# RS2002/PianoBart

Measured on AMD Instinct MI355X. Metric: Octuple tokens/sec/GPU (seq=1024, 12L/768d) pretrain step; %MFMA peak, higher is better.
Workload: dtype bf16

## Files before the change

pianobart_amd/csrc/pb_fa_tiles.h:

```cpp
#pragma once
#include "pb_common.h"
#include "pb_api_internal.h"

namespace {


constexpr int HD = 64, FT = 256;
constexpr float LOG2E = 1.4426950408889634f;
typedef __attribute__((ext_vector_type(4))) short s16x4;
typedef __attribute__((ext_vector_type(8))) short s16x8;

struct Fa64Args {
    const bf16_t *q, *k, *v, *o, *dout;
    bf16_t *out, *dq, *dk, *dv;
    float* lse; const float* delta; const float* key_mask; const int* kmax;
    int B, H, Sq, Sk;
    long q_sb, q_ss, k_sb, k_ss, v_sb, v_ss, o_sb, o_ss, dq_sb, dq_ss, dk_sb, dk_ss, dv_sb, dv_ss;
    float scale; int causal;
    float* cs_q; float* cs_kv;
    const bf16_t* zeros;
    const int *vl_q_off, *vl_k_off, *vl_q_len, *vl_k_len;
    const int* bh_order;
};

inline Fa64Args fa64_args(const pb_attn_desc& d, bool bwd) {
    Fa64Args a = {};
    a.q = (const bf16_t*)d.q; a.k = (const bf16_t*)d.k; a.v = (const bf16_t*)d.v; a.dout = (const bf16_t*)d.dout;
    if (bwd) a.o = (const bf16_t*)d.o; else a.out = (bf16_t*)d.o;
    a.dq = (bf16_t*)d.dq; a.dk = (bf16_t*)d.dk; a.dv = (bf16_t*)d.dv; a.lse = d.lse; a.delta = d.delta;
    a.key_mask = d.key_mask; a.kmax = d.q_off ? d.k_vis : d.kmax;
    a.B = d.B; a.H = d.H; a.Sq = d.Sq; a.Sk = d.Sk;
    a.q_sb = d.q_sb; a.q_ss = d.q_ss; a.k_sb = d.k_sb; a.k_ss = d.k_ss; a.v_sb = d.v_sb; a.v_ss = d.v_ss; a.o_sb = d.o_sb; a.o_ss = d.o_ss;
    a.dq_sb = d.dq_sb; a.dq_ss = d.dq_ss; a.dk_sb = d.dk_sb; a.dk_ss = d.dk_ss; a.dv_sb = d.dv_sb; a.dv_ss = d.dv_ss;
    a.scale = d.scale; a.causal = d.flags & PB_ATTN_CAUSAL;
    a.zeros = (const bf16_t*)pb_zero_page();
    a.vl_q_off = d.q_off; a.vl_k_off = d.k_off; a.vl_q_len = d.q_len; a.vl_k_len = d.k_len; a.bh_order = d.bh_order;
    return a;
}

__device__ __forceinline__ void varlen_localize(Fa64Args& p, int b) {
    if (!p.vl_q_off) return;
    const long qo = p.vl_q_off[b], ko = p.vl_k_off[b];
    p.Sq = p.vl_q_len[b]; p.Sk = p.vl_k_len[b];
    p.q += qo * p.q_ss - b * p.q_sb; p.k += ko * p.k_ss - b * p.k_sb; p.v += ko * p.v_ss - b * p.v_sb;
    if (p.o) p.o += qo * p.o_ss - b * p.o_sb;
    if (p.out) p.out += qo * p.o_ss - b * p.o_sb;
    if (p.dout) p.dout += qo * p.o_ss - b * p.o_sb;
    if (p.dq) p.dq += qo * p.dq_ss - b * p.dq_sb;
    if (p.dk) p.dk += ko * p.dk_ss - b * p.dk_sb;
    if (p.dv) p.dv += ko * p.dv_ss - b * p.dv_sb;
}

#define MFMA16(a, b, c) __builtin_amdgcn_mfma_f32_16x16x32_bf16((a), (b), (c), 0, 0, 0)

__device__ __forceinline__ int fsw(int row) { return (((row >> 1) & 3) << 1) | ((row >> 3) & 1); }

__device__ __forceinline__ void glds16(const bf16_t* g, char* lds_wave_base) {
    __builtin_amdgcn_global_load_lds((const __attribute__((address_space(1))) void*)g,
                                     (__attribute__((address_space(3))) void*)lds_wave_base, 16, 0, 0);
}
struct StageOff { unsigned off[2]; unsigned chunk[2]; };
__device__ __forceinline__ StageOff stage_off(long ld, int wave, int lane) {
    StageOff o;
#pragma unroll
    for (int n = 0; n < 2; ++n) {
        const int row = (wave * 2 + n) * 8 + (lane >> 3);
        o.chunk[n] = (unsigned)((lane & 7) ^ fsw(row));
        o.off[n] = (unsigned)(row * ld + (o.chunk[n] << 3));
    }
    return o;
}
__device__ __forceinline__ void stage64(const bf16_t* __restrict__ base, long ld, int r0, int nrows, char* lds, int wave, int lane, const StageOff& so,
                                        int cmax = 8, const bf16_t* zeros = nullptr) {
    if (r0 + 64 <= nrows) {
        const bf16_t* tb = base + (long)r0 * ld;
#pragma unroll
        for (int n = 0; n < 2; ++n) glds16((cmax == 8 || (int)so.chunk[n] < cmax) ? tb + so.off[n] : zeros, lds + (wave * 2 + n) * 1024);
    } else {
#pragma unroll
        for (int n = 0; n < 2; ++n) {
            const int inst = wave * 2 + n;
            const int row = inst * 8 + (lane >> 3);
            const int chunk = (lane & 7) ^ fsw(row);
            const int gr = min(r0 + row, nrows - 1);
            glds16((cmax == 8 || chunk < cmax) ? base + (long)gr * ld + chunk * 8 : zeros, lds + inst * 1024);
        }
    }
}
__device__ __forceinline__ bf16x8 frag_row(const char* lds, int row, int ks, int g) {
    return *reinterpret_cast<const bf16x8*>(lds + row * 128 + (((ks * 4 + g) ^ fsw(row)) << 4));
}
__device__ __forceinline__ bf16x8 frag_tr(const char* lds, int c0, int s, int lane) {
    const int lr = lane & 15, g = lane >> 4, qq = lr >> 2, pp = lr & 3;
    const int chunk = (c0 >> 3) + (pp >> 1);
    const int r0 = 32 * s + 4 * g + qq, r1 = r0 + 16;
    const int o0 = r0 * 128 + ((chunk ^ fsw(r0)) << 4) + ((pp & 1) << 3);
    const int o1 = r1 * 128 + ((chunk ^ fsw(r1)) << 4) + ((pp & 1) << 3);
    const s16x4 lo = __builtin_amdgcn_ds_read_tr16_b64_v4i16((__attribute__((address_space(3))) s16x4*)(lds + o0));
    const s16x4 hi = __builtin_amdgcn_ds_read_tr16_b64_v4i16((__attribute__((address_space(3))) s16x4*)(lds + o1));
    const s16x8 v = {lo[0], lo[1], lo[2], lo[3], hi[0], hi[1], hi[2], hi[3]};
    return __builtin_bit_cast(bf16x8, v);
}
__device__ __forceinline__ bf16x8 pack_pair(const f32x4& lo, const f32x4& hi) {
    bf16x8 r = {(bf16_t)lo[0], (bf16_t)lo[1], (bf16_t)lo[2], (bf16_t)lo[3], (bf16_t)hi[0], (bf16_t)hi[1], (bf16_t)hi[2], (bf16_t)hi[3]};
    return r;
}
__device__ __forceinline__ bf16x8 frag_global(const bf16_t* __restrict__ g, long ld, int row, int nvalid, int col) {
    bf16x8 z = {};
    if (row < nvalid) z = *reinterpret_cast<const bf16x8*>(g + (long)row * ld + col);
    return z;
}
__device__ __forceinline__ float grp_max(float v) {
    auto a = __builtin_amdgcn_permlane16_swap(__float_as_uint(v), __float_as_uint(v), false, false);
    v = fmaxf(__uint_as_float(a[0]), __uint_as_float(a[1]));
    auto b = __builtin_amdgcn_permlane32_swap(__float_as_uint(v), __float_as_uint(v), false, false);
    return fmaxf(__uint_as_float(b[0]), __uint_as_float(b[1]));
}
__device__ __forceinline__ float grp_sum(float v) {
    auto a = __builtin_amdgcn_permlane16_swap(__float_as_uint(v), __float_as_uint(v), false, false);
    v = __uint_as_float(a[0]) + __uint_as_float(a[1]);
    auto b = __builtin_amdgcn_permlane32_swap(__float_as_uint(v), __float_as_uint(v), false, false);
    return __uint_as_float(b[0]) + __uint_as_float(b[1]);
}
template <bool V> struct BoolTag { static constexpr bool value = V; };

constexpr int STG = 2 * 8192 + 512;
// ... 54 lines not shown
```

pianobart_amd/csrc/pb_flash1.hip:

```cpp
#include "pb_common.h"
#include "pb_fa_tiles.h"
#include <cstdlib>
#include <algorithm>

namespace {

constexpr int KB1 = 256;
constexpr int RING1 = 3, STB1 = 2 * 8192;
constexpr int OFF_K = RING1 * STB1;
constexpr int OFF_DS = OFF_K + 4 * 8192;
constexpr int OFF_TAB = OFF_DS + 2 * 2 * 8192;

struct Fa1Args {
    Fa64Args a;
    bf16_t* slab;
    long slab_stride, slab_sb;
    const float* delta_rows; long delta_ld;
    unsigned* stamps;
};

#define PB_U10(p) p "0", p "1", p "2", p "3", p "4", p "5", p "6", p "7", p "8", p "9"
#define PB_ALL_AGPRS PB_U10("a"), PB_U10("a1"), PB_U10("a2"), PB_U10("a3"), PB_U10("a4"), PB_U10("a5"), PB_U10("a6"), PB_U10("a7"), PB_U10("a8"), PB_U10("a9"), \
    PB_U10("a10"), PB_U10("a11"), PB_U10("a12"), PB_U10("a13"), PB_U10("a14"), PB_U10("a15"), PB_U10("a16"), PB_U10("a17"), PB_U10("a18"), PB_U10("a19"), \
    PB_U10("a20"), PB_U10("a21"), PB_U10("a22"), PB_U10("a23"), PB_U10("a24"), "a250", "a251", "a252", "a253", "a254", "a255"
constexpr int A_DK = 0, A_DV = 64, A_KF = 128, A_VF = 160, A_KT = 192;
typedef __attribute__((ext_vector_type(4))) unsigned u32x4;

template <int R> __device__ __forceinline__ void agpr_zero() { asm volatile("v_accvgpr_write_b32 a%c0, 0" :: "i"(R)); }
template <int R> __device__ __forceinline__ void agpr_put(const bf16x8& v) {
    const u32x4 u = __builtin_bit_cast(u32x4, v);
    asm volatile("v_accvgpr_write_b32 a%c4, %0\n\tv_accvgpr_write_b32 a%c5, %1\n\tv_accvgpr_write_b32 a%c6, %2\n\tv_accvgpr_write_b32 a%c7, %3"
                 :: "v"(u[0]), "v"(u[1]), "v"(u[2]), "v"(u[3]), "i"(R), "i"(R + 1), "i"(R + 2), "i"(R + 3));
}
template <int R> __device__ __forceinline__ f32x4 agpr_get() {
    f32x4 r;
    asm volatile("v_accvgpr_read_b32 %0, a%c4\n\tv_accvgpr_read_b32 %1, a%c5\n\tv_accvgpr_read_b32 %2, a%c6\n\tv_accvgpr_read_b32 %3, a%c7"
                 : "=v"(r[0]), "=v"(r[1]), "=v"(r[2]), "=v"(r[3]) : "i"(R), "i"(R + 1), "i"(R + 2), "i"(R + 3));
    return r;
}
template <int RB> __device__ __forceinline__ void mfma_vab_c(f32x4& d, const bf16x8& a, const f32x4& c) {
    asm volatile("v_mfma_f32_16x16x32_bf16 %0, %1, a[%c3:%c4], %2" : "=&v"(d) : "v"(a), "v"(c), "i"(RB), "i"(RB + 3) : PB_ALL_AGPRS);
}
template <int RB> __device__ __forceinline__ void mfma_vab(f32x4& d, const bf16x8& a) {
    asm volatile("v_mfma_f32_16x16x32_bf16 %0, %1, a[%c2:%c3], %0" : "+v"(d) : "v"(a), "i"(RB), "i"(RB + 3) : PB_ALL_AGPRS);
}
template <int RA> __device__ __forceinline__ void mfma_aav(f32x4& d, const bf16x8& b) {
    asm volatile("v_mfma_f32_16x16x32_bf16 %0, a[%c2:%c3], %1, %0" : "+v"(d) : "v"(b), "i"(RA), "i"(RA + 3) : PB_ALL_AGPRS);
}
template <int RA> __device__ __forceinline__ void mfma_aav_z(f32x4& d, const bf16x8& b) {
    asm volatile("v_mfma_f32_16x16x32_bf16 %0, a[%c2:%c3], %1, 0" : "=&v"(d) : "v"(b), "i"(RA), "i"(RA + 3) : PB_ALL_AGPRS);
}
template <int RD> __device__ __forceinline__ void mfma_acc(const bf16x8& b, const bf16x8& a) {
    asm volatile("v_mfma_f32_16x16x32_bf16 a[%c2:%c3], %0, %1, a[%c2:%c3]" :: "v"(a), "v"(b), "i"(RD), "i"(RD + 3) : PB_ALL_AGPRS);
}
#define MF "v_mfma_f32_16x16x32_bf16 "
template <int DT, int K0> __device__ __forceinline__ void mfma_dvdk4(const bf16x8& p0, const bf16x8& d0, const bf16x8& p1, const bf16x8& d1, const bf16x8& ot, const bf16x8& qt) {
    asm volatile(MF "a[%c6:%c7], %4, %0, a[%c6:%c7]\n\t" MF "a[%c8:%c9], %5, %1, a[%c8:%c9]\n\t" MF "a[%c10:%c11], %4, %2, a[%c10:%c11]\n\t" MF "a[%c12:%c13], %5, %3, a[%c12:%c13]"
                 :: "v"(p0), "v"(d0), "v"(p1), "v"(d1), "v"(ot), "v"(qt),
                    "i"(A_DV + 4 * (K0 * 4 + DT)), "i"(A_DV + 4 * (K0 * 4 + DT) + 3), "i"(A_DK + 4 * (K0 * 4 + DT)), "i"(A_DK + 4 * (K0 * 4 + DT) + 3),
                    "i"(A_DV + 4 * ((K0 + 1) * 4 + DT)), "i"(A_DV + 4 * ((K0 + 1) * 4 + DT) + 3), "i"(A_DK + 4 * ((K0 + 1) * 4 + DT)), "i"(A_DK + 4 * ((K0 + 1) * 4 + DT) + 3)
                 : PB_ALL_AGPRS);
}
template <int KT> __device__ __forceinline__ void mfma_sdp0(f32x4& sv, f32x4& dp, const bf16x8& qa, const bf16x8& oa, const f32x4& nl, const f32x4& nd) {
    asm volatile(MF "%0, %2, a[%c6:%c7], %4\n\t" MF "%1, %3, a[%c8:%c9], %5"
                 : "=&v"(sv), "=&v"(dp) : "v"(qa), "v"(oa), "v"(nl), "v"(nd),
                   "i"(A_KF + 4 * (KT * 2)), "i"(A_KF + 4 * (KT * 2) + 3), "i"(A_VF + 4 * (KT * 2)), "i"(A_VF + 4 * (KT * 2) + 3) : PB_ALL_AGPRS);
}
template <int KT> __device__ __forceinline__ void mfma_sdp1(f32x4& sv, f32x4& dp, const bf16x8& qa, const bf16x8& oa) {
    asm volatile(MF "%0, %2, a[%c4:%c5], %0\n\t" MF "%1, %3, a[%c6:%c7], %1"
                 : "+v"(sv), "+v"(dp) : "v"(qa), "v"(oa),
                   "i"(A_KF + 4 * (KT * 2 + 1)), "i"(A_KF + 4 * (KT * 2 + 1) + 3), "i"(A_VF + 4 * (KT * 2 + 1)), "i"(A_VF + 4 * (KT * 2 + 1) + 3) : PB_ALL_AGPRS);
}
template <int S0, bool ZERO> __device__ __forceinline__ void mfma_dq4(f32x4& a0, f32x4& b0, f32x4& a1, f32x4& b1, const bf16x8& bs0, const bf16x8& bs1) {
    if constexpr (ZERO)
        asm volatile(MF "%0, a[%c6:%c7], %4, 0\n\t" MF "%1, a[%c8:%c9], %4, 0\n\t" MF "%2, a[%c10:%c11], %5, 0\n\t" MF "%3, a[%c12:%c13], %5, 0"
                     : "=&v"(a0), "=&v"(b0), "=&v"(a1), "=&v"(b1) : "v"(bs0), "v"(bs1),
                       "i"(A_KT + 4 * S0), "i"(A_KT + 4 * S0 + 3), "i"(A_KT + 4 * (8 + S0)), "i"(A_KT + 4 * (8 + S0) + 3),
                       "i"(A_KT + 4 * (S0 + 1)), "i"(A_KT + 4 * (S0 + 1) + 3), "i"(A_KT + 4 * (9 + S0)), "i"(A_KT + 4 * (9 + S0) + 3) : PB_ALL_AGPRS);
    else
        asm volatile(MF "%0, a[%c6:%c7], %4, %0\n\t" MF "%1, a[%c8:%c9], %4, %1\n\t" MF "%2, a[%c10:%c11], %5, %2\n\t" MF "%3, a[%c12:%c13], %5, %3"
                     : "+v"(a0), "+v"(b0), "+v"(a1), "+v"(b1) : "v"(bs0), "v"(bs1),
                       "i"(A_KT + 4 * S0), "i"(A_KT + 4 * S0 + 3), "i"(A_KT + 4 * (8 + S0)), "i"(A_KT + 4 * (8 + S0) + 3),
                       "i"(A_KT + 4 * (S0 + 1)), "i"(A_KT + 4 * (S0 + 1) + 3), "i"(A_KT + 4 * (9 + S0)), "i"(A_KT + 4 * (9 + S0) + 3) : PB_ALL_AGPRS);
}
#undef MF
template <int OFF, class T> __device__ __forceinline__ void ds_rd128(T& d, unsigned addr) {
    static_assert(sizeof(T) == 16, "16-byte fragment");
    asm volatile("ds_read_b128 %0, %1 offset:%2" : "=v"(d) : "v"(addr), "i"(OFF));
}
__device__ __forceinline__ bf16x4 to_bf4(const f32x4& v) {
    bf16x4 r = {(bf16_t)v[0], (bf16_t)v[1], (bf16_t)v[2], (bf16_t)v[3]};
    return r;
}
__device__ __forceinline__ bf16x8 join4(const bf16x4& lo, const bf16x4& hi) { return __builtin_shufflevector(lo, hi, 0, 1, 2, 3, 4, 5, 6, 7); }
#define PB_PIN() __builtin_amdgcn_sched_barrier(0)

__global__ __launch_bounds__(FT) void fa1_bwd_kernel(const Fa1Args pin) {
    constexpr int HDT = 64;
    extern __shared__ __attribute__((aligned(16))) char smem[];
    const int t = threadIdx.x, lane = t & 63, lr = lane & 15, g = lane >> 4;
    const int wave = __builtin_amdgcn_readfirstlane(t >> 6);
#ifdef PB_FA1_STAMPS
    const unsigned long long st_in = __builtin_amdgcn_s_memrealtime();
#endif
    const int nkb0 = (pin.a.Sk + KB1 - 1) / KB1;
    int rb, h, b;
    block_map(nkb0, pin.a.H, pin.a.B, rb, h, b, pin.a.bh_order);
    const int k0 = rb * KB1;
    Fa64Args p = pin.a;
    const long qrow0 = pin.a.vl_q_off ? (long)pin.a.vl_q_off[b] : (long)b * pin.a.Sq;
    varlen_localize(p, b);
    const int lse_ld = pin.a.Sq, d_model = p.H * HDT;
    const int kvis_end = p.kmax ? min(p.Sk, p.kmax[b]) : p.Sk;
    const int nt = (p.Sq + 63) / 64;
    const int it0 = p.causal ? k0 / 64 : 0;
    const bf16_t* K = p.k + b * p.k_sb + h * HDT;
    const bf16_t* V = p.v + b * p.v_sb + h * HDT;
    if (k0 >= kvis_end || it0 >= nt) {
        for (int i = t; i < KB1 * 8; i += FT) {
            const int key = k0 + (i >> 3), ch = i & 7;
            if (key < p.Sk) {
                const bf16x8 z = {};
                *reinterpret_cast<bf16x8*>(p.dk + b * p.dk_sb + (long)key * p.dk_ss + h * HDT + ch * 8) = z;
                *reinterpret_cast<bf16x8*>(p.dv + b * p.dv_sb + (long)key * p.dv_ss + h * HDT + ch * 8) = z;
            }
        }
        if (p.cs_kv && t < 2 * HDT) {
            float* row = p.cs_kv + (long)(b * nkb0 + rb) * 2 * d_model + h * HDT;
            row[t < HDT ? t : d_model + t - HDT] = 0.f;
        }
        return;
    }
    asm volatile("" ::: PB_ALL_AGPRS);
#ifdef PB_FA1_STAMPS
    const unsigned st_t0 = (unsigned)__builtin_amdgcn_s_memtime();
    unsigned st_p[6] = {}, st_q[4] = {};
#define PSTAMP(i) st_p[i] = (unsigned)__builtin_amdgcn_s_memtime();
#define QSTAMP(i) st_q[i] = (unsigned)__builtin_amdgcn_s_memtime();
#else
#define PSTAMP(i)
#define QSTAMP(i)
#endif
    const bf16_t* Q = p.q + b * p.q_sb + h * HDT;
    const bf16_t* DO = p.dout + b * p.o_sb + h * HDT;
    bf16_t* slab = pin.slab + (long)rb * pin.slab_stride + (pin.a.vl_q_off ? qrow0 * d_model : (long)b * pin.slab_sb) + h * HDT;
    const float c = p.scale * LOG2E;
    bf16x8 kfr[4][2], vfr[4][2];
#pragma unroll
    for (int kt = 0; kt < 4; ++kt) {
        const int key = k0 + wave * 64 + kt * 16 + lr;
#pragma unroll
        for (int ks = 0; ks < 2; ++ks) {
            kfr[kt][ks] = frag_global(K, p.k_ss, key, p.Sk, ks * 32 + g * 8);
            vfr[kt][ks] = frag_global(V, p.v_ss, key, p.Sk, ks * 32 + g * 8);
        }
    }
    QSTAMP(0);
    float* ldsNL = reinterpret_cast<float*>(smem + OFF_TAB);
    float* ldsND = ldsNL + nt * 64;
    float* ldsVis = reinterpret_cast<float*>(smem + OFF_DS);
    const long li0 = ((long)b * p.H + h) * lse_ld;
    const float* dsrc = pin.delta_rows ? pin.delta_rows + (long)h * pin.delta_ld + qrow0 : p.delta + li0;
    float tl[4], td[4];
#pragma unroll
    for (int i = 0; i < 4; ++i) {
        const int q = it0 * 64 + t + i * FT;
        tl[i] = q < p.Sq ? p.lse[li0 + q] : INFINITY;
        td[i] = q < p.Sq ? dsrc[q] : 0.f;
    }
    QSTAMP(1);
    const int key_t = k0 + t;
    const float vis_t = (key_t < kvis_end && (!p.key_mask || p.key_mask[(long)b * p.Sk + key_t] != 0.f)) ? 1.f : 0.f;
    const StageOff so_k = stage_off(p.k_ss, wave, lane), so_q = stage_off(p.q_ss, wave, lane), so_o = stage_off(p.o_ss, wave, lane);
    const __amdgpu_buffer_rsrc_t rsK = __builtin_amdgcn_make_buffer_rsrc(const_cast<bf16_t*>(K), 0, (int)(((long)(p.Sk - 1) * p.k_ss + HDT) * 2), 0x00020000);
    const __amdgpu_buffer_rsrc_t rsQ = __builtin_amdgcn_make_buffer_rsrc(const_cast<bf16_t*>(Q), 0, (int)(((long)(p.Sq - 1) * p.q_ss + HDT) * 2), 0x00020000);
    const __amdgpu_buffer_rsrc_t rsO = __builtin_amdgcn_make_buffer_rsrc(const_cast<bf16_t*>(DO), 0, (int)(((long)(p.Sq - 1) * p.o_ss + HDT) * 2), 0x00020000);
    const __amdgpu_buffer_rsrc_t rsS = __builtin_amdgcn_make_buffer_rsrc(slab, 0, (int)(((long)(p.Sq - 1) * d_model + HDT) * 2), 0x00020000);
    const unsigned stg = lds_u32(smem) + OFF_K + (unsigned)(wave * 1024);
    const unsigned stg_wa = stg + (unsigned)(lr * 64 + ((((g >> 1) ^ ((lr >> 1) & 3)) << 4) | ((g & 1) << 3)));
    const unsigned stg_wb = stg + (unsigned)(lr * 64 + (((2 + (g >> 1)) ^ ((lr >> 1) & 3)) << 4 | ((g & 1) << 3)));
    const int srow = lane >> 2, schunk = lane & 3;
    const unsigned stg_rd = stg + (unsigned)(srow * 64 + ((schunk ^ ((srow >> 1) & 3)) << 4));
    const unsigned slab_vo = (unsigned)((((wave & 1) * 16 + srow) * d_model + (wave >> 1) * 32 + schunk * 8) * 2);
    u32x4 slab_v = {0u, 0u, 0u, 0u};
    int slab_qs = 0;
    bool slab_pending = false;
    typedef __attribute__((ext_vector_type(2))) unsigned u32x2_t;
    auto slab_put = [&](const f32x4& a, const f32x4& b_, int qs) {
        *reinterpret_cast<__attribute__((address_space(3))) u32x2_t*>(stg_wa) = __builtin_bit_cast(u32x2_t, to_bf4(a));
        *reinterpret_cast<__attribute__((address_space(3))) u32x2_t*>(stg_wb) = __builtin_bit_cast(u32x2_t, to_bf4(b_));
        ds_rd128<0>(slab_v, stg_rd);
        slab_qs = qs; slab_pending = true;
    };
    auto slab_flush = [&]() {
        if (slab_pending) { __builtin_amdgcn_raw_buffer_store_b128(slab_v, rsS, slab_vo, slab_qs, 0); slab_pending = false; }
    };
    const unsigned voQ0 = so_q.off[0] * 2, voQ1 = so_q.off[1] * 2, voO0 = so_o.off[0] * 2, voO1 = so_o.off[1] * 2;
    typedef __attribute__((address_space(3))) void* lds_t;
#pragma unroll
    for (int m = 0; m < 4; ++m) {
        const int sk = (k0 + 64 * m) * (int)p.k_ss * 2;
        __builtin_amdgcn_raw_ptr_buffer_load_lds(rsK, (lds_t)(smem + OFF_K + m * 8192 + wave * 2048), 16, so_k.off[0] * 2, sk, 0, 0);
        __builtin_amdgcn_raw_ptr_buffer_load_lds(rsK, (lds_t)(smem + OFF_K + m * 8192 + wave * 2048 + 1024), 16, so_k.off[1] * 2, sk, 0, 0);
    }
    auto stage = [&](int it, int slot) {
        char* st = smem + slot * STB1 + wave * 2048;
        const int sq = it * 64 * (int)p.q_ss * 2, so = it * 64 * (int)p.o_ss * 2;
        __builtin_amdgcn_raw_ptr_buffer_load_lds(rsQ, (lds_t)st, 16, voQ0, sq, 0, 0);
        __builtin_amdgcn_raw_ptr_buffer_load_lds(rsQ, (lds_t)(st + 1024), 16, voQ1, sq, 0, 0);
        __builtin_amdgcn_raw_ptr_buffer_load_lds(rsO, (lds_t)(st + 8192), 16, voO0, so, 0, 0);
        __builtin_amdgcn_raw_ptr_buffer_load_lds(rsO, (lds_t)(st + 8192 + 1024), 16, voO1, so, 0, 0);
    };
    QSTAMP(2);
    const int npre = min(3, nt - it0);
    stage(it0, 0);
    if (npre > 1) stage(it0 + 1, 1);
    if (npre > 2) stage(it0 + 2, 2);
    PSTAMP(0);
#pragma unroll
    for (int i = 0; i < 4; ++i) {
        const int q = it0 * 64 + t + i * FT;
        if (q < nt * 64) { ldsNL[q] = tl[i] == INFINITY ? -INFINITY : -tl[i] * LOG2E; ldsND[q] = -td[i]; }
    }
    for (int q = it0 * 64 + t + 4 * FT; q < nt * 64; q += FT) {
        const float ls = q < p.Sq ? p.lse[li0 + q] : INFINITY;
        ldsNL[q] = ls == INFINITY ? -INFINITY : -ls * LOG2E;
        ldsND[q] = q < p.Sq ? -dsrc[q] : 0.f;
    }
    ldsVis[t] = vis_t;
    bool hot = false;
#pragma unroll
    for (int i = 0; i < 4; ++i) hot |= (tl[i] != INFINITY && -tl[i] * LOG2E > 100.f);
    for (int q = it0 * 64 + t + 4 * FT; q < p.Sq; q += FT) hot |= (-p.lse[li0 + q] * LOG2E > 100.f);
    unsigned* ldsHot = reinterpret_cast<unsigned*>(smem + OFF_DS + 1024);
    const unsigned hotw = __builtin_amdgcn_ballot_w64(hot) != 0ull ? 1u : 0u;
    if (lane == 0) ldsHot[wave] = hotw;
    PSTAMP(1);
    bool allvis = true;
    static_for<0, 4>([&](auto ktt) {
        constexpr int kt = decltype(ktt)::value;
        const int key = k0 + wave * 64 + kt * 16 + lr;
        const bool vis = key < kvis_end && (!p.key_mask || p.key_mask[(long)b * p.Sk + key] != 0.f);
        allvis &= vis;
        static_for<0, 2>([&](auto kss) {
            constexpr int ks = decltype(kss)::value;
            bf16x8 kf = scale_frag(kfr[kt][ks], c);
            const bf16x8 z = {};
            if (!vis) kf = z;
            agpr_put<A_KF + 4 * (kt * 2 + ks)>(kf);
            agpr_put<A_VF + 4 * (kt * 2 + ks)>(vfr[kt][ks]);
        });
    });
    static_for<0, 128>([&](auto r) { agpr_zero<decltype(r)::value>(); });
    PSTAMP(2);
    asm volatile("s_waitcnt vmcnt(0)" ::: "memory");
    PSTAMP(3);
    __builtin_amdgcn_s_waitcnt(0xc07f);
    __builtin_amdgcn_s_barrier();
    const bool careful = __builtin_amdgcn_ballot_w64(!allvis) != 0ull &&
                         __builtin_amdgcn_readfirstlane(ldsHot[0] | ldsHot[1] | ldsHot[2] | ldsHot[3]) != 0u;
    PSTAMP(4);
    const int qsel = wave & 1, cpair = wave >> 1;
    {
        s16x4 tk[2][4][2][2];
#pragma unroll
        for (int ct = 0; ct < 2; ++ct)
#pragma unroll
            for (int m = 0; m < 4; ++m) ds_tr_block(tk[ct][m], lds_u32(smem) + OFF_K + m * 8192 + tr_lane_off64((cpair * 2 + ct) * 16, lane));
        tr_wait8(tk[0], tk[1]);
        static_for<0, 8>([&](auto ss) {
            constexpr int s = decltype(ss)::value;
            const f32x4 m0 = *reinterpret_cast<const f32x4*>(ldsVis + 32 * s + 4 * g), m1 = *reinterpret_cast<const f32x4*>(ldsVis + 32 * s + 16 + 4 * g);
            static_for<0, 2>([&](auto ctt) {
                constexpr int ct = decltype(ctt)::value;
                bf16x8 f = tr_join(tk[ct][s >> 1][s & 1][0], tk[ct][s >> 1][s & 1][1]);
#pragma unroll
                for (int j = 0; j < 4; ++j) { if (m0[j] == 0.f) f[j] = (bf16_t)0.f; if (m1[j] == 0.f) f[4 + j] = (bf16_t)0.f; }
                agpr_put<A_KT + 4 * (ct * 8 + s)>(f);
            });
        });
    }
    PSTAMP(5);
    unsigned qoff[4];
#pragma unroll
    for (int dt = 0; dt < 4; ++dt) qoff[dt] = lds_u32(smem) + tr_lane_off64(dt * 16, lane);
    unsigned frow[2];
#pragma unroll
    for (int ks = 0; ks < 2; ++ks) frow[ks] = lds_u32(smem) + (unsigned)(lr * 128 + (((ks * 4 + g) ^ fsw(lr)) << 4));
    const unsigned tab_nl = lds_u32(smem) + OFF_TAB + (unsigned)(g * 16), tab_nd = tab_nl + (unsigned)(nt * 256);
    const unsigned ds_wr = lds_u32(smem) + OFF_DS + (unsigned)((wave * 64 + lr) * 32 + ((g ^ (lr >> 2)) << 3));
    const unsigned ds_rd = lds_u32(smem) + OFF_DS + (unsigned)(qsel * 8192 + (4 * g + (lr >> 2)) * 32 + (((lr & 3) ^ g) << 3));
    if (npre == 3) { wait_vm<8>(); } else if (npre == 2) { wait_vm<4>(); } else { wait_vm<0>(); }
    __builtin_amdgcn_s_waitcnt(0xc07f);
    __builtin_amdgcn_s_barrier();

    bf16x8 pfp[4], dfp[4];
    s16x4 to[2][2], tq[2][2];
    const int mykey0 = k0 + wave * 64 + lr;

#ifdef PB_FA1_STAMPS
    unsigned st_acc[12] = {}, st_last = 0, st_steps = 0;
#endif
#if defined(PB_FA1_STAMPS) && PB_FA1_STAMPS > 1
#define STAMP(i) { const unsigned now_ = (unsigned)__builtin_amdgcn_s_memtime(); st_acc[i] += now_ - st_last; st_last = now_; }
#else
#define STAMP(i)
#endif
    auto step = [&](int T, int slot, int pslot, int stage_tile, auto halftag, auto firsttag, auto diagtag) {
        constexpr int HALF = decltype(halftag)::value;
        constexpr bool FIRST = decltype(firsttag)::value != 0, DIAG = decltype(diagtag)::value != 0;
        constexpr int PH = 1 - HALF;
        constexpr int qtA = HALF * 2, qtB = HALF * 2 + 1;
        const int q0 = T * 64;
        const unsigned fq0 = frow[0] + (unsigned)(slot * STB1), fq1 = frow[1] + (unsigned)(slot * STB1);
        const unsigned tnl = tab_nl + (unsigned)(q0 * 4), tnd = tab_nd + (unsigned)(q0 * 4);
        f32x4 nlA, ndA, nlB, ndB;
        bf16x8 qaA0, oaA0, qaA1, oaA1, qaB0, oaB0, qaB1, oaB1;
        STAMP(0);
        ds_rd128<qtA * 64>(nlA, tnl); ds_rd128<qtA * 64>(ndA, tnd);
        ds_rd128<qtA * 2048>(qaA0, fq0); ds_rd128<qtA * 2048 + 8192>(oaA0, fq0); ds_rd128<qtA * 2048>(qaA1, fq1); ds_rd128<qtA * 2048 + 8192>(oaA1, fq1);
        s16x4 to2[2][2], tq2[2][2];
        if constexpr (!FIRST) {
            const bf16x8 ot0 = tr_join(to[0][0], to[0][1]), qt0 = tr_join(tq[0][0], tq[0][1]);
            mfma_dvdk4<0, 0>(pfp[0], dfp[0], pfp[1], dfp[1], ot0, qt0);
#pragma unroll
            for (int d2 = 0; d2 < 2; ++d2) {
                const unsigned aq = qoff[2 + d2] + (unsigned)((HALF ? slot : pslot) * STB1), ao = aq + 8192;
                if constexpr (PH == 0) { ds_tr<0>(to2[d2][0], ao); ds_tr<2048>(to2[d2][1], ao); ds_tr<0>(tq2[d2][0], aq); ds_tr<2048>(tq2[d2][1], aq); }
                else { ds_tr<4096>(to2[d2][0], ao); ds_tr<6144>(to2[d2][1], ao); ds_tr<4096>(tq2[d2][0], aq); ds_tr<6144>(tq2[d2][1], aq); }
            }
            mfma_dvdk4<0, 2>(pfp[2], dfp[2], pfp[3], dfp[3], ot0, qt0);
            if (stage_tile >= 0) stage(stage_tile, pslot);
            const bf16x8 ot1 = tr_join(to[1][0], to[1][1]), qt1 = tr_join(tq[1][0], tq[1][1]);
            mfma_dvdk4<1, 0>(pfp[0], dfp[0], pfp[1], dfp[1], ot1, qt1);
            mfma_dvdk4<1, 2>(pfp[2], dfp[2], pfp[3], dfp[3], ot1, qt1);
            STAMP(1);
            asm volatile("s_waitcnt lgkmcnt(8)" : "+v"(nlA), "+v"(ndA), "+v"(qaA0), "+v"(oaA0), "+v"(qaA1), "+v"(oaA1));
            STAMP(2);
        } else {
            asm volatile("s_waitcnt lgkmcnt(0)" : "+v"(nlA), "+v"(ndA), "+v"(qaA0), "+v"(oaA0), "+v"(qaA1), "+v"(oaA1));
        }
        f32x4 svA[4], dpA[4], svB[4], dpB[4];
        static_for<0, 4>([&](auto ktt) { constexpr int kt = decltype(ktt)::value; mfma_sdp0<kt>(svA[kt], dpA[kt], qaA0, oaA0, nlA, ndA); });
        ds_rd128<qtB * 64>(nlB, tnl); ds_rd128<qtB * 64>(ndB, tnd);
        ds_rd128<qtB * 2048>(qaB0, fq0); ds_rd128<qtB * 2048 + 8192>(oaB0, fq0); ds_rd128<qtB * 2048>(qaB1, fq1); ds_rd128<qtB * 2048 + 8192>(oaB1, fq1);
        static_for<0, 4>([&](auto ktt) { constexpr int kt = decltype(ktt)::value; mfma_sdp1<kt>(svA[kt], dpA[kt], qaA1, oaA1); });
        STAMP(3);
        if constexpr (!FIRST)
            asm volatile("s_waitcnt lgkmcnt(0)" : "+v"(nlB), "+v"(ndB), "+v"(qaB0), "+v"(oaB0), "+v"(qaB1), "+v"(oaB1),
                                                  "+v"(to2[0][0]), "+v"(to2[0][1]), "+v"(to2[1][0]), "+v"(to2[1][1]), "+v"(tq2[0][0]), "+v"(tq2[0][1]), "+v"(tq2[1][0]), "+v"(tq2[1][1]));
        else
            asm volatile("s_waitcnt lgkmcnt(0)" : "+v"(nlB), "+v"(ndB), "+v"(qaB0), "+v"(oaB0), "+v"(qaB1), "+v"(oaB1));
        auto next_tr = [&]() {
#pragma unroll
            for (int dt = 0; dt < 2; ++dt) {
                const unsigned aq = qoff[dt] + (unsigned)(slot * STB1), ao = aq + 8192;
                if constexpr (HALF == 0) { ds_tr<0>(to[dt][0], ao); ds_tr<2048>(to[dt][1], ao); ds_tr<0>(tq[dt][0], aq); ds_tr<2048>(tq[dt][1], aq); }
                else { ds_tr<4096>(to[dt][0], ao); ds_tr<6144>(to[dt][1], ao); ds_tr<4096>(tq[dt][0], aq); ds_tr<6144>(tq[dt][1], aq); }
            }
        };
        unsigned pw[4][2][2], dw[4][2][2];
        STAMP(4);
        const unsigned wr = ds_wr + HALF * 16384;
// ... 126 lines not shown
        ds_tr<4096>(sb[4][0], base); ds_tr<4608>(sb[4][1], base); ds_tr<5120>(sb[5][0], base); ds_tr<5632>(sb[5][1], base);
        ds_tr<6144>(sb[6][0], base); ds_tr<6656>(sb[6][1], base); ds_tr<7168>(sb[7][0], base); ds_tr<7680>(sb[7][1], base);
        s16x4 to2[2][2], tq2[2][2];
#pragma unroll
        for (int d2 = 0; d2 < 2; ++d2) {
            const unsigned aq = qoff[2 + d2] + (unsigned)(slot * STB1), ao = aq + 8192;
            ds_tr<4096>(to2[d2][0], ao); ds_tr<6144>(to2[d2][1], ao); ds_tr<4096>(tq2[d2][0], aq); ds_tr<6144>(tq2[d2][1], aq);
        }
        static_for<0, 2>([&](auto dtt) {
            constexpr int dt = decltype(dtt)::value;
            const bf16x8 ot = tr_join(to[dt][0], to[dt][1]), qt = tr_join(tq[dt][0], tq[dt][1]);
            static_for<0, 4>([&](auto ktt) {
                constexpr int kt = decltype(ktt)::value;
                mfma_acc<A_DV + 4 * (kt * 4 + dt)>(pfp[kt], ot);
                mfma_acc<A_DK + 4 * (kt * 4 + dt)>(dfp[kt], qt);
            });
        });
        asm volatile("s_waitcnt lgkmcnt(0)" : "+v"(to2[0][0]), "+v"(to2[0][1]), "+v"(to2[1][0]), "+v"(to2[1][1]), "+v"(tq2[0][0]), "+v"(tq2[0][1]), "+v"(tq2[1][0]), "+v"(tq2[1][1]));
        static_for<0, 2>([&](auto dtt) {
            constexpr int dt = 2 + decltype(dtt)::value;
            const bf16x8 ot = tr_join(to2[dt - 2][0], to2[dt - 2][1]), qt = tr_join(tq2[dt - 2][0], tq2[dt - 2][1]);
            static_for<0, 4>([&](auto ktt) {
                constexpr int kt = decltype(ktt)::value;
                mfma_acc<A_DV + 4 * (kt * 4 + dt)>(pfp[kt], ot);
                mfma_acc<A_DK + 4 * (kt * 4 + dt)>(dfp[kt], qt);
            });
        });
        asm volatile("s_waitcnt lgkmcnt(0)" : "+v"(sb[0][0]), "+v"(sb[0][1]), "+v"(sb[1][0]), "+v"(sb[1][1]), "+v"(sb[2][0]), "+v"(sb[2][1]), "+v"(sb[3][0]), "+v"(sb[3][1]),
                                              "+v"(sb[4][0]), "+v"(sb[4][1]), "+v"(sb[5][0]), "+v"(sb[5][1]), "+v"(sb[6][0]), "+v"(sb[6][1]), "+v"(sb[7][0]), "+v"(sb[7][1]));
        f32x4 dqa, dqb;
        static_for<0, 8>([&](auto ss) {
            constexpr int s = decltype(ss)::value;
            const bf16x8 bs = tr_join(sb[s][0], sb[s][1]);
            if constexpr (s == 0) { mfma_aav_z<A_KT>(dqa, bs); mfma_aav_z<A_KT + 32>(dqb, bs); }
            else { mfma_aav<A_KT + 4 * s>(dqa, bs); mfma_aav<A_KT + 4 * (8 + s)>(dqb, bs); }
        });
        asm volatile("s_nop 15" : "+v"(dqa), "+v"(dqb));
        typedef __attribute__((ext_vector_type(2))) unsigned u32x2;
        const int qs = (T * 64 + 32) * d_model * 2;
        slab_put(dqa * p.scale, dqb * p.scale, qs);
        asm volatile("s_waitcnt lgkmcnt(0)" : "+v"(slab_v) :: "memory");
        slab_flush();
    }

    asm volatile("s_nop 15\n\ts_nop 7" ::: "memory");
#ifdef PB_FA1_STAMPS
    const unsigned st_e0 = (unsigned)__builtin_amdgcn_s_memtime();
#endif
    f32x4 csk[4], csv[4];
#pragma unroll
    for (int dt = 0; dt < 4; ++dt) { csk[dt] = f32x4{0.f, 0.f, 0.f, 0.f}; csv[dt] = f32x4{0.f, 0.f, 0.f, 0.f}; }
    static_for<0, 4>([&](auto ktt) {
        constexpr int kt = decltype(ktt)::value;
        const int key = k0 + wave * 64 + kt * 16 + lr;
        const bool kvis = key < kvis_end && (!p.key_mask || p.key_mask[(long)b * p.Sk + (key < p.Sk ? key : 0)] != 0.f);
        bf16_t* DK = p.dk + b * p.dk_sb + (long)key * p.dk_ss + h * HDT + (g >> 1) * 8;
        bf16_t* DV = p.dv + b * p.dv_sb + (long)key * p.dv_ss + h * HDT + (g >> 1) * 8;
        static_for<0, 2>([&](auto dpp) {
            constexpr int dt0 = 2 * decltype(dpp)::value, dt1 = dt0 + 1;
            f32x4 vk0 = agpr_get<A_DK + 4 * (kt * 4 + dt0)>() * p.scale, vv0 = agpr_get<A_DV + 4 * (kt * 4 + dt0)>();
            f32x4 vk1 = agpr_get<A_DK + 4 * (kt * 4 + dt1)>() * p.scale, vv1 = agpr_get<A_DV + 4 * (kt * 4 + dt1)>();
            if (!kvis) { vk0 = vv0 = vk1 = vv1 = f32x4{0.f, 0.f, 0.f, 0.f}; }
            csk[dt0] += vk0; csv[dt0] += vv0; csk[dt1] += vk1; csv[dt1] += vv1;
            typedef __attribute__((ext_vector_type(2))) unsigned u32x2;
            auto pair16 = [&](const f32x4& x, const f32x4& y) {
                const u32x2 xu = __builtin_bit_cast(u32x2, to_bf4(x)), yu = __builtin_bit_cast(u32x2, to_bf4(y));
                const auto s0 = __builtin_amdgcn_permlane16_swap(xu[0], yu[0], false, false);
                const auto s1 = __builtin_amdgcn_permlane16_swap(xu[1], yu[1], false, false);
                const u32x4 r = {s0[0], s1[0], s0[1], s1[1]};
                return r;
            };
            const u32x4 rk = pair16(vk0, vk1), rv = pair16(vv0, vv1);
            if (key < p.Sk) {
                const int col = ((g & 1) ? dt1 : dt0) * 16;
                *reinterpret_cast<u32x4*>(DK + col) = rk;
                *reinterpret_cast<u32x4*>(DV + col) = rv;
            }
        });
    });
#ifdef PB_FA1_STAMPS
    const unsigned st_e1 = (unsigned)__builtin_amdgcn_s_memtime();
#endif
    if (p.cs_kv) {
        float* red = reinterpret_cast<float*>(smem);
        __syncthreads();
#pragma unroll
        for (int dt = 0; dt < 4; ++dt) {
#pragma unroll
            for (int e = 0; e < 4; ++e) {
                float v = csk[dt][e], u = csv[dt][e];
                v += PB_DPP_F(v, 0x140); u += PB_DPP_F(u, 0x140);
                v += PB_DPP_F(v, 0x141); u += PB_DPP_F(u, 0x141);
                v += PB_DPP_F(v, 0x4e); u += PB_DPP_F(u, 0x4e);
                v += PB_DPP_F(v, 0xb1); u += PB_DPP_F(u, 0xb1);
                csk[dt][e] = v; csv[dt][e] = u;
            }
            if (lr == 0) {
                *reinterpret_cast<f32x4*>(red + wave * 2 * HDT + dt * 16 + g * 4) = csk[dt];
                *reinterpret_cast<f32x4*>(red + wave * 2 * HDT + HDT + dt * 16 + g * 4) = csv[dt];
            }
        }
        __syncthreads();
        if (t < 2 * HDT) {
            float* row = p.cs_kv + (long)(b * nkb0 + rb) * 2 * d_model + h * HDT;
            const float v = red[t] + red[2 * HDT + t] + red[4 * HDT + t] + red[6 * HDT + t];
            row[t < HDT ? t : d_model + t - HDT] = v;
        }
    }
#ifdef PB_FA1_STAMPS
    if (pin.stamps && lane == 0) {
        const unsigned st_t3 = (unsigned)__builtin_amdgcn_s_memtime();
        const unsigned ntrace = pin.stamps[32];
        if (ntrace) {
            if (wave == 0 && blockIdx.x < ntrace) {
                unsigned hw, xcc;
                asm volatile("s_getreg_b32 %0, hwreg(HW_REG_HW_ID)" : "=s"(hw));
                asm volatile("s_getreg_b32 %0, hwreg(HW_REG_XCC_ID)" : "=s"(xcc));
                const unsigned long long st_out = __builtin_amdgcn_s_memrealtime();
                unsigned long long* rec = reinterpret_cast<unsigned long long*>(pin.stamps + 64) + 4 * (size_t)blockIdx.x;
                rec[0] = ((unsigned long long)(xcc & 15) << 32) | hw; rec[1] = st_in; rec[2] = st_out;
                rec[3] = ((unsigned long long)(st_t1 - st_t0) << 32) | (unsigned)(st_t3 - st_t2);
            }
        } else {
        for (int i = 0; i < 10; ++i) atomicAdd(pin.stamps + i, st_acc[i] >> 4);
        atomicAdd(pin.stamps + 16, st_steps);
        atomicAdd(pin.stamps + 10, (st_t1 - st_t0) >> 4); atomicAdd(pin.stamps + 11, (st_t2 - st_t1) >> 4); atomicAdd(pin.stamps + 12, (st_t3 - st_t2) >> 4);
        atomicAdd(pin.stamps + 17, 1u);
        atomicAdd(pin.stamps + 18, (st_p[0] - st_t0) >> 4); atomicAdd(pin.stamps + 19, (st_p[1] - st_p[0]) >> 4); atomicAdd(pin.stamps + 20, (st_p[2] - st_p[1]) >> 4);
        atomicAdd(pin.stamps + 21, (st_p[3] - st_p[2]) >> 4); atomicAdd(pin.stamps + 22, (st_p[4] - st_p[3]) >> 4); atomicAdd(pin.stamps + 23, (st_p[5] - st_p[4]) >> 4);
        atomicAdd(pin.stamps + 24, (st_t1 - st_p[5]) >> 4);
        atomicAdd(pin.stamps + 28, (st_q[0] - st_t0) >> 4); atomicAdd(pin.stamps + 29, (st_q[1] - st_q[0]) >> 4); atomicAdd(pin.stamps + 30, (st_q[2] - st_q[1]) >> 4); atomicAdd(pin.stamps + 31, (st_p[0] - st_q[2]) >> 4);
        atomicAdd(pin.stamps + 25, (st_e0 - st_t2) >> 4); atomicAdd(pin.stamps + 26, (st_e1 - st_e0) >> 4); atomicAdd(pin.stamps + 27, (st_t3 - st_e1) >> 4);
        }
    }
#endif
}

__global__ __launch_bounds__(256) void fa1_delta_kernel(const Fa64Args pin, int rows_per_block) {
    const int b = blockIdx.y;
    Fa64Args p = pin;
    varlen_localize(p, b);
    const int lse_ld = pin.Sq, H = p.H, G = H * 8;
    const int s0 = blockIdx.x * rows_per_block, s1 = min(p.Sq, s0 + rows_per_block);
    for (int i = threadIdx.x; i < (s1 - s0) * G; i += 256) {
        const int s = s0 + i / G, j = i % G;
        const bf16x8 a = *reinterpret_cast<const bf16x8*>(p.dout + b * p.o_sb + (long)s * p.o_ss + j * 8);
        const bf16x8 o = *reinterpret_cast<const bf16x8*>(p.o + b * p.o_sb + (long)s * p.o_ss + j * 8);
        float acc = 0.f;
#pragma unroll
        for (int e = 0; e < 8; ++e) acc = fmaf((float)a[e], (float)o[e], acc);
        acc += PB_DPP_F(acc, 0xb1);
        acc += PB_DPP_F(acc, 0x4e);
        acc += PB_DPP_F(acc, 0x141);
        if ((j & 7) == 0) const_cast<float*>(p.delta)[((long)b * H + (j >> 3)) * lse_ld + s] = acc;
    }
}

constexpr int RCH = 64;
__global__ __launch_bounds__(1024) void fa1_reduce_kernel(const Fa1Args pin, int RL) {
    extern __shared__ __attribute__((aligned(16))) char smem[];
    const int b = blockIdx.y, chunk = blockIdx.x;
    Fa64Args p = pin.a;
    varlen_localize(p, b);
    const int d_model = p.H * 64, G = p.H * 8;
    const int nch = (pin.a.Sq + RCH - 1) / RCH;
    const int kvis_end = p.kmax ? min(p.Sk, p.kmax[b]) : p.Sk;
    const int nvalid = (kvis_end + KB1 - 1) / KB1;
    const bf16_t* slab = pin.slab + (pin.a.vl_q_off ? (long)pin.a.vl_q_off[b] * d_model : (long)b * pin.slab_sb);
    const int cg = threadIdx.x % G, rl = threadIdx.x / G;
    float cs[8];
#pragma unroll
    for (int e = 0; e < 8; ++e) cs[e] = 0.f;
    const int s1 = min(p.Sq, chunk * RCH + RCH);
    auto row = [&](int s) {
        const int nb = p.causal ? min(nvalid, s / KB1 + 1) : nvalid;
        bf16x8 v[4];
#pragma unroll
        for (int j = 0; j < 4; ++j) if (j < nb) v[j] = *reinterpret_cast<const bf16x8*>(slab + (long)j * pin.slab_stride + (long)s * d_model + cg * 8);
        float acc[8];
#pragma unroll
        for (int e = 0; e < 8; ++e) acc[e] = 0.f;
#pragma unroll
        for (int j = 0; j < 4; ++j) if (j < nb) {
#pragma unroll
            for (int e = 0; e < 8; ++e) acc[e] += (float)v[j][e];
        }
        for (int j = 4; j < nb; ++j) {
            const bf16x8 w = *reinterpret_cast<const bf16x8*>(slab + (long)j * pin.slab_stride + (long)s * d_model + cg * 8);
#pragma unroll
            for (int e = 0; e < 8; ++e) acc[e] += (float)w[e];
        }
        bf16x8 r;
#pragma unroll
        for (int e = 0; e < 8; ++e) { r[e] = (bf16_t)acc[e]; cs[e] += (float)r[e]; }
        *reinterpret_cast<bf16x8*>(p.dq + b * p.dq_sb + (long)s * p.dq_ss + cg * 8) = r;
    };
    if (rl < RL) {
        int s = chunk * RCH + rl;
        for (; s + RL < s1; s += 2 * RL) { row(s); row(s + RL); }
        if (s < s1) row(s);
    }
    if (p.cs_q) {
        float* red = reinterpret_cast<float*>(smem);
        if (rl < RL)
// ... 63 lines not shown
```

Measured before the change: 627,900.

## Restructure FA1 backward prologue: LDS K fragments, batched scalar loads, deferred staging

The flash-attention backward prologue now reads the K fragments from the staged LDS tile instead of from global memory, and batches the varlen and kmax scalar loads into a single s_load group with one wait. Visibility per key comes from ds_bpermute of an existing visibility value. Staging of the next two Q tiles is deferred until after the K setup, and the per-column masking of the transposed K is skipped when the block is fully visible. The cs_kv reduction reuses a different LDS region so one barrier can be dropped, and the timing-stamp records are extended. The goal is to shorten the prologue latency before the main loop. The cost is extra complexity and a risk of LDS hazards in the aliasing and staging order.

```diff
diff --git a/pianobart_amd/csrc/pb_fa_tiles.h b/pianobart_amd/csrc/pb_fa_tiles.h
--- a/pianobart_amd/csrc/pb_fa_tiles.h
+++ b/pianobart_amd/csrc/pb_fa_tiles.h
@@ -42,6 +42,16 @@
     if (!p.vl_q_off) return;
     const long qo = p.vl_q_off[b], ko = p.vl_k_off[b];
     p.Sq = p.vl_q_len[b]; p.Sk = p.vl_k_len[b];
+    p.q += qo * p.q_ss - b * p.q_sb; p.k += ko * p.k_ss - b * p.k_sb; p.v += ko * p.v_ss - b * p.v_sb;
+    if (p.o) p.o += qo * p.o_ss - b * p.o_sb;
+    if (p.out) p.out += qo * p.o_ss - b * p.o_sb;
+    if (p.dout) p.dout += qo * p.o_ss - b * p.o_sb;
+    if (p.dq) p.dq += qo * p.dq_ss - b * p.dq_sb;
+    if (p.dk) p.dk += ko * p.dk_ss - b * p.dk_sb;
+    if (p.dv) p.dv += ko * p.dv_ss - b * p.dv_sb;
+}
+__device__ __forceinline__ void varlen_apply(Fa64Args& p, int b, long qo, long ko, int q_len, int k_len) {
+    p.Sq = q_len; p.Sk = k_len;
     p.q += qo * p.q_ss - b * p.q_sb; p.k += ko * p.k_ss - b * p.k_sb; p.v += ko * p.v_ss - b * p.v_sb;
     if (p.o) p.o += qo * p.o_ss - b * p.o_sb;
     if (p.out) p.out += qo * p.o_ss - b * p.o_sb;
diff --git a/pianobart_amd/csrc/pb_flash1.hip b/pianobart_amd/csrc/pb_flash1.hip
--- a/pianobart_amd/csrc/pb_flash1.hip
+++ b/pianobart_amd/csrc/pb_flash1.hip
@@ -102,16 +102,24 @@
     const int wave = __builtin_amdgcn_readfirstlane(t >> 6);
 #ifdef PB_FA1_STAMPS
     const unsigned long long st_in = __builtin_amdgcn_s_memrealtime();
+    const unsigned st_in32 = (unsigned)__builtin_amdgcn_s_memtime();
 #endif
     const int nkb0 = (pin.a.Sk + KB1 - 1) / KB1;
     int rb, h, b;
     block_map(nkb0, pin.a.H, pin.a.B, rb, h, b, pin.a.bh_order);
     const int k0 = rb * KB1;
     Fa64Args p = pin.a;
-    const long qrow0 = pin.a.vl_q_off ? (long)pin.a.vl_q_off[b] : (long)b * pin.a.Sq;
-    varlen_localize(p, b);
+    const int* zi = reinterpret_cast<const int*>(pin.a.zeros);
+    const bool vl = pin.a.vl_q_off != nullptr;
+    int w_qo, w_ko, w_ql, w_kl, w_km;
+    asm volatile("s_load_dword %0, %5, 0x0\n\ts_load_dword %1, %6, 0x0\n\ts_load_dword %2, %7, 0x0\n\ts_load_dword %3, %8, 0x0\n\ts_load_dword %4, %9, 0x0\n\ts_waitcnt lgkmcnt(0)"
+                 : "=&s"(w_qo), "=&s"(w_ko), "=&s"(w_ql), "=&s"(w_kl), "=&s"(w_km)
+                 : "s"(vl ? pin.a.vl_q_off + b : zi), "s"(vl ? pin.a.vl_k_off + b : zi), "s"(vl ? pin.a.vl_q_len + b : zi), "s"(vl ? pin.a.vl_k_len + b : zi), "s"(pin.a.kmax ? pin.a.kmax + b : zi)
+                 : "memory");
+    const long qrow0 = vl ? (long)w_qo : (long)b * pin.a.Sq;
+    if (vl) varlen_apply(p, b, w_qo, w_ko, w_ql, w_kl);
     const int lse_ld = pin.a.Sq, d_model = p.H * HDT;
-    const int kvis_end = p.kmax ? min(p.Sk, p.kmax[b]) : p.Sk;
+    const int kvis_end = p.kmax ? min(p.Sk, w_km) : p.Sk;
     const int nt = (p.Sq + 63) / 64;
     const int it0 = p.causal ? k0 / 64 : 0;
     const bf16_t* K = p.k + b * p.k_sb + h * HDT;
@@ -145,15 +153,12 @@
     const bf16_t* DO = p.dout + b * p.o_sb + h * HDT;
     bf16_t* slab = pin.slab + (long)rb * pin.slab_stride + (pin.a.vl_q_off ? qrow0 * d_model : (long)b * pin.slab_sb) + h * HDT;
     const float c = p.scale * LOG2E;
-    bf16x8 kfr[4][2], vfr[4][2];
+    bf16x8 vfr[4][2];
 #pragma unroll
     for (int kt = 0; kt < 4; ++kt) {
         const int key = k0 + wave * 64 + kt * 16 + lr;
 #pragma unroll
-        for (int ks = 0; ks < 2; ++ks) {
-            kfr[kt][ks] = frag_global(K, p.k_ss, key, p.Sk, ks * 32 + g * 8);
-            vfr[kt][ks] = frag_global(V, p.v_ss, key, p.Sk, ks * 32 + g * 8);
-        }
+        for (int ks = 0; ks < 2; ++ks) vfr[kt][ks] = frag_global(V, p.v_ss, key, p.Sk, ks * 32 + g * 8);
     }
     QSTAMP(0);
     float* ldsNL = reinterpret_cast<float*>(smem + OFF_TAB);
@@ -214,9 +219,8 @@
     QSTAMP(2);
     const int npre = min(3, nt - it0);
     stage(it0, 0);
-    if (npre > 1) stage(it0 + 1, 1);
-    if (npre > 2) stage(it0 + 2, 2);
     PSTAMP(0);
+    static_for<0, 128>([&](auto r) { agpr_zero<decltype(r)::value>(); });
 #pragma unroll
     for (int i = 0; i < 4; ++i) {
         const int q = it0 * 64 + t + i * FT;
@@ -236,24 +240,15 @@
     const unsigned hotw = __builtin_amdgcn_ballot_w64(hot) != 0ull ? 1u : 0u;
     if (lane == 0) ldsHot[wave] = hotw;
     PSTAMP(1);
-    bool allvis = true;
+    bool allvis = true, visk[4];
     static_for<0, 4>([&](auto ktt) {
         constexpr int kt = decltype(ktt)::value;
-        const int key = k0 + wave * 64 + kt * 16 + lr;
-        const bool vis = key < kvis_end && (!p.key_mask || p.key_mask[(long)b * p.Sk + key] != 0.f);
-        allvis &= vis;
-        static_for<0, 2>([&](auto kss) {
-            constexpr int ks = decltype(kss)::value;
-            bf16x8 kf = scale_frag(kfr[kt][ks], c);
-            const bf16x8 z = {};
-            if (!vis) kf = z;
-            agpr_put<A_KF + 4 * (kt * 2 + ks)>(kf);
-            agpr_put<A_VF + 4 * (kt * 2 + ks)>(vfr[kt][ks]);
-        });
+        visk[kt] = __builtin_amdgcn_ds_bpermute((kt * 16 + lr) << 2, __float_as_int(vis_t)) != 0;
+        allvis &= visk[kt];
+        static_for<0, 2>([&](auto kss) { constexpr int ks = decltype(kss)::value; agpr_put<A_VF + 4 * (kt * 2 + ks)>(vfr[kt][ks]); });
     });
-    static_for<0, 128>([&](auto r) { agpr_zero<decltype(r)::value>(); });
     PSTAMP(2);
-    asm volatile("s_waitcnt vmcnt(0)" ::: "memory");
+    wait_vm<4>();
     PSTAMP(3);
     __builtin_amdgcn_s_waitcnt(0xc07f);
     __builtin_amdgcn_s_barrier();
@@ -261,24 +256,51 @@
                          __builtin_amdgcn_readfirstlane(ldsHot[0] | ldsHot[1] | ldsHot[2] | ldsHot[3]) != 0u;
     PSTAMP(4);
     const int qsel = wave & 1, cpair = wave >> 1;
+    const bool fullblk = !p.key_mask && k0 + KB1 <= kvis_end;
     {
+        if (fullblk) { if (npre > 1) stage(it0 + 1, 1); if (npre > 2) stage(it0 + 2, 2); }
+        bf16x8 kfr[4][2];
         s16x4 tk[2][4][2][2];
+        const unsigned krow = lds_u32(smem) + OFF_K + (unsigned)(wave * 8192 + lr * 128);
+        const unsigned kc0 = (unsigned)((g ^ fsw(lr)) << 4), kc1 = (unsigned)(((4 + g) ^ fsw(lr)) << 4);
+        ds_rd128<0>(kfr[0][0], krow + kc0); ds_rd128<0>(kfr[0][1], krow + kc1); ds_rd128<2048>(kfr[1][0], krow + kc0); ds_rd128<2048>(kfr[1][1], krow + kc1);
+        ds_rd128<4096>(kfr[2][0], krow + kc0); ds_rd128<4096>(kfr[2][1], krow + kc1); ds_rd128<6144>(kfr[3][0], krow + kc0); ds_rd128<6144>(kfr[3][1], krow + kc1);
 #pragma unroll
         for (int ct = 0; ct < 2; ++ct)
 #pragma unroll
             for (int m = 0; m < 4; ++m) ds_tr_block(tk[ct][m], lds_u32(smem) + OFF_K + m * 8192 + tr_lane_off64((cpair * 2 + ct) * 16, lane));
+        asm volatile("s_waitcnt lgkmcnt(0)" : "+v"(kfr[0][0]), "+v"(kfr[0][1]), "+v"(kfr[1][0]), "+v"(kfr[1][1]), "+v"(kfr[2][0]), "+v"(kfr[2][1]), "+v"(kfr[3][0]), "+v"(kfr[3][1]));
         tr_wait8(tk[0], tk[1]);
-        static_for<0, 8>([&](auto ss) {
-            constexpr int s = decltype(ss)::value;
-            const f32x4 m0 = *reinterpret_cast<const f32x4*>(ldsVis + 32 * s + 4 * g), m1 = *reinterpret_cast<const f32x4*>(ldsVis + 32 * s + 16 + 4 * g);
-            static_for<0, 2>([&](auto ctt) {
-                constexpr int ct = decltype(ctt)::value;
-                bf16x8 f = tr_join(tk[ct][s >> 1][s & 1][0], tk[ct][s >> 1][s & 1][1]);
-#pragma unroll
-                for (int j = 0; j < 4; ++j) { if (m0[j] == 0.f) f[j] = (bf16_t)0.f; if (m1[j] == 0.f) f[4 + j] = (bf16_t)0.f; }
-                agpr_put<A_KT + 4 * (ct * 8 + s)>(f);
+        static_for<0, 4>([&](auto ktt) {
+            constexpr int kt = decltype(ktt)::value;
+            static_for<0, 2>([&](auto kss) {
+                constexpr int ks = decltype(kss)::value;
+                bf16x8 kf = scale_frag(kfr[kt][ks], c);
+                const bf16x8 z = {};
+                if (!visk[kt]) kf = z;
+                agpr_put<A_KF + 4 * (kt * 2 + ks)>(kf);
             });
         });
+        if (fullblk) {
+            static_for<0, 8>([&](auto ss) {
+                constexpr int s = decltype(ss)::value;
+                static_for<0, 2>([&](auto ctt) { constexpr int ct = decltype(ctt)::value; agpr_put<A_KT + 4 * (ct * 8 + s)>(tr_join(tk[ct][s >> 1][s & 1][0], tk[ct][s >> 1][s & 1][1])); });
+            });
+        } else {
+            static_for<0, 8>([&](auto ss) {
+                constexpr int s = decltype(ss)::value;
+                const f32x4 m0 = *reinterpret_cast<const f32x4*>(ldsVis + 32 * s + 4 * g), m1 = *reinterpret_cast<const f32x4*>(ldsVis + 32 * s + 16 + 4 * g);
+                static_for<0, 2>([&](auto ctt) {
+                    constexpr int ct = decltype(ctt)::value;
+                    bf16x8 f = tr_join(tk[ct][s >> 1][s & 1][0], tk[ct][s >> 1][s & 1][1]);
+#pragma unroll
+                    for (int j = 0; j < 4; ++j) { if (m0[j] == 0.f) f[j] = (bf16_t)0.f; if (m1[j] == 0.f) f[4 + j] = (bf16_t)0.f; }
+                    agpr_put<A_KT + 4 * (ct * 8 + s)>(f);
+                });
+            });
+            if (npre > 1) stage(it0 + 1, 1);
+            if (npre > 2) stage(it0 + 2, 2);
+        }
     }
     PSTAMP(5);
     unsigned qoff[4];
@@ -571,8 +593,7 @@
     const unsigned st_e1 = (unsigned)__builtin_amdgcn_s_memtime();
 #endif
     if (p.cs_kv) {
-        float* red = reinterpret_cast<float*>(smem);
-        __syncthreads();
+        float* red = reinterpret_cast<float*>(smem + OFF_K + 4096);
 #pragma unroll
         for (int dt = 0; dt < 4; ++dt) {
 #pragma unroll
@@ -589,7 +610,8 @@
                 *reinterpret_cast<f32x4*>(red + wave * 2 * HDT + HDT + dt * 16 + g * 4) = csv[dt];
             }
         }
-        __syncthreads();
+        __builtin_amdgcn_s_waitcnt(0xc07f);
+        __builtin_amdgcn_s_barrier();
         if (t < 2 * HDT) {
             float* row = p.cs_kv + (long)(b * nkb0 + rb) * 2 * d_model + h * HDT;
             const float v = red[t] + red[2 * HDT + t] + red[4 * HDT + t] + red[6 * HDT + t];
@@ -606,9 +628,12 @@
                 asm volatile("s_getreg_b32 %0, hwreg(HW_REG_HW_ID)" : "=s"(hw));
                 asm volatile("s_getreg_b32 %0, hwreg(HW_REG_XCC_ID)" : "=s"(xcc));
                 const unsigned long long st_out = __builtin_amdgcn_s_memrealtime();
-                unsigned long long* rec = reinterpret_cast<unsigned long long*>(pin.stamps + 64) + 4 * (size_t)blockIdx.x;
+                unsigned long long* rec = reinterpret_cast<unsigned long long*>(pin.stamps + 64) + 16 * (size_t)blockIdx.x;
                 rec[0] = ((unsigned long long)(xcc & 15) << 32) | hw; rec[1] = st_in; rec[2] = st_out;
                 rec[3] = ((unsigned long long)(st_t1 - st_t0) << 32) | (unsigned)(st_t3 - st_t2);
+                const unsigned ph[14] = {st_q[0] - st_t0, st_q[1] - st_q[0], st_q[2] - st_q[1], st_p[0] - st_q[2], st_p[1] - st_p[0], st_p[2] - st_p[1], st_p[3] - st_p[2],
+                                         st_p[4] - st_p[3], st_p[5] - st_p[4], st_t1 - st_p[5], st_e0 - st_t2, st_e1 - st_e0, st_t3 - st_e1, st_t0 - st_in32};
+                for (int i = 0; i < 7; ++i) rec[4 + i] = ((unsigned long long)ph[2 * i + 1] << 32) | ph[2 * i];
             }
         } else {
         for (int i = 0; i < 10; ++i) atomicAdd(pin.stamps + i, st_acc[i] >> 4);
```

Result: no change. 631,800, median of 6 (+0.6%).
